# Chrixtar/latentsplat

Measured on AMD Instinct MI355X. Metric: rendered target views/sec at 256x256, ~300k Gaussians (forward); fwd+bwd ms/view in `fwdbwd`, higher is better.
Workload: dtype f32; 1 GPU; BASELINE configs[1]: 300000 latent Gaussians (4-ch features + opacity), 256x256, forward render; 16 views of one scene per step per GPU; gaussians=300000, parallelism=replicas x1 (one scene per rank, no data-path collective)

## Files before the change

latentsplat_amd/csrc/binning.hip:

```cpp
#include "lsr_blend.h"
#include "lsr_tile_scan.h"
#include <algorithm>
#include <mutex>
#ifdef LSR_ENABLE_TRACE
#include <cstdio>
#include <cstdlib>
#include <vector>
#endif

namespace lsr {

constexpr int kScanThreads = 1024;

constexpr int kScanRegs = 8;

__global__ void __launch_bounds__(kScanThreads)
k_tile_scan(const uint32_t *__restrict__ count, uint32_t *__restrict__ start, uint32_t *header,
            uint32_t *host_words, uint32_t host_seq, uint32_t *__restrict__ order, int N, uint32_t capacity) {
    __shared__ TileScanShared<kScanThreads> s_scan;
    tile_scan_block<kScanThreads, kScanRegs, false>(count, start, header, HostMirror{host_words, host_seq}, order, N, capacity, s_scan);
}

hipError_t launch_tile_scan(const lsr_dims &d, char *geom, uint32_t *host_words, uint32_t host_seq, uint32_t pair_capacity, hipStream_t s) {
    const GeomLayout L = geom_layout(d);
    const int N = d.num_views * (int)num_tiles(d);
    prof_begin(kStTileScan, s);
    hipLaunchKernelGGL(k_tile_scan, dim3(1), dim3(kScanThreads), 0, s,
                       (const uint32_t *)(geom + L.tile_count), (uint32_t *)(geom + L.tile_start),
                       (uint32_t *)(geom + L.header), host_words, host_seq, (uint32_t *)(geom + L.tile_order), N, pair_capacity);
    prof_end(kStTileScan, s);
    return hipGetLastError();
}

constexpr int kScatThreads = 256;
constexpr int kScatItems = 12;

template <bool LDS_RESERVE, bool NARROW>
__global__ void __launch_bounds__(kScatThreads, NARROW ? 8 : 6)
k_scatter(int G, int gx, int T, const char *__restrict__ binrec,
          const uint32_t *__restrict__ tile_start, uint32_t *__restrict__ tile_cursor,
          uint64_t *__restrict__ keys, uint32_t capacity, uint32_t chunks, int items, uint32_t key_shift, unsigned long long *trace,
          const uint32_t *__restrict__ tile_count, const uint32_t *__restrict__ header, uint32_t over_cap, int skip_none) {
    if (over_cap && header[kHdrMaxTile] <= over_cap) return;
#ifdef LSR_ENABLE_TRACE
#define LSR_STAMP(k) do { if (trace && threadIdx.x == 0) trace[8 * (size_t)blockIdx.x + (k)] = wall_clock64(); } while (0)
#else
#define LSR_STAMP(k) do { } while (0)
#endif
    LSR_STAMP(0);
    extern __shared__ uint32_t s_mem[];
    uint32_t *s_cnt = s_mem, *s_base = s_mem + T;
    const uint32_t unit = blockIdx.x;
    const int v = (int)(unit / chunks);
    const size_t vo = (size_t)v * G;
    const uint32_t *ts = tile_start + (size_t)v * T;
    uint32_t *cur = tile_cursor + (size_t)v * T;
    const uint32_t *tcv = tile_count + (size_t)v * T;
    const int base = (int)(unit % chunks) * (kScatThreads * items);
    uint32_t lo16[kScatItems], hi16[NARROW ? 1 : kScatItems], span[kScatItems];
    float dep[kScatItems];
#pragma unroll
    for (int it = 0; it < kScatItems; ++it) {
        const int i = base + min(it, items - 1) * kScatThreads + (int)threadIdx.x;
        const bool valid = it < items && i < G;
        if (NARROW) {
            const uint3 br = *(const uint3 *)(binrec + (vo + min(i, G - 1)) * sizeof(BinRec));
            lo16[it] = valid ? br.x : 0u; dep[it] = __uint_as_float(br.y); span[it] = br.z;
        } else {
            const uint4 br = *(const uint4 *)(binrec + (vo + min(i, G - 1)) * sizeof(BinRecWide));
            lo16[it] = br.x; hi16[NARROW ? 0 : it] = valid ? br.y : 0u; dep[it] = __uint_as_float(br.z); span[it] = br.w;
        }
    }
    auto unpack = [&](int it, int &x0, int &y0, int &x1, int &y1) {
        uint32_t a = lo16[it], b = NARROW ? 0u : hi16[NARROW ? 0 : it];
        asm volatile("" : "+v"(a), "+v"(b));
        if (NARROW) { x0 = a & 0xff; y0 = (a >> 8) & 0xff; x1 = (a >> 16) & 0xff; y1 = a >> 24; }
        else { x0 = a & 0xffff; y0 = a >> 16; x1 = b & 0xffff; y1 = b >> 16; }
    };
    if (LDS_RESERVE) {
        for (int t = threadIdx.x; t < T; t += kScatThreads) s_cnt[t] = 0;
        __syncthreads();
        LSR_STAMP(1);
#pragma unroll
        for (int it = 0; it < kScatItems; ++it) {
            int x0, y0, x1, y1;
            unpack(it, x0, y0, x1, y1);
            if (skip_none) reached_rect(span[it], x0, y0, x1, y1);
            for (int y = y0; y < y1; ++y)
                for (int x = x0; x < x1; ++x) {
                    if (over_cap && tcv[y * gx + x] <= over_cap) continue;
                    atomicAdd(&s_cnt[y * gx + x], 1u);
                }
        }
        __syncthreads();
        LSR_STAMP(2);
        for (int t = threadIdx.x; t < T; t += kScatThreads) {
            const uint32_t c = s_cnt[t];
            if (c) s_base[t] = ts[t] + atomicAdd(&cur[t], c);
            s_cnt[t] = 0;
        }
        __syncthreads();
        LSR_STAMP(3);
    }
    uint32_t tid2 = threadIdx.x;
    asm volatile("" : "+v"(tid2));
#pragma unroll
    for (int it = 0; it < kScatItems; ++it) {
        const uint32_t i = (uint32_t)(base + it * kScatThreads) + tid2;
        int x0, y0, x1, y1;
        unpack(it, x0, y0, x1, y1);
        if (x1 <= x0 || y1 <= y0) continue;
        const uint64_t key = ((uint64_t)__float_as_uint(dep[it]) << 32) | (i << key_shift);
        const uint32_t sp = span[it];
        int ex0 = x0, ey0 = y0, ex1 = x1, ey1 = y1;
        if (skip_none) reached_rect(sp, ex0, ey0, ex1, ey1);
        for (int y = ey0; y < ey1; ++y)
            for (int x = ex0; x < ex1; ++x) {
                const int t = y * gx + x;
                if (over_cap && tcv[t] <= over_cap) continue;
                const uint32_t code = key_shift ? span_code(sp, x - x0, y - y0) : 0u;
                uint32_t pos;
                if (LDS_RESERVE) pos = s_base[t] + atomicAdd(&s_cnt[t], 1u);
                else pos = ts[t] + atomicAdd(&cur[t], 1u);
                keys[min(pos, capacity - 1u)] = key | code;
            }
    }
    LSR_STAMP(4);
#ifdef LSR_ENABLE_TRACE
    __builtin_amdgcn_s_waitcnt(0);
    __syncthreads();
    LSR_STAMP(5);
    if (trace && threadIdx.x == 0) {
        unsigned hwid, xcc;
        asm volatile("s_getreg_b32 %0, hwreg(HW_REG_HW_ID)" : "=s"(hwid));
        asm volatile("s_getreg_b32 %0, hwreg(HW_REG_XCC_ID)" : "=s"(xcc));
        trace[8 * (size_t)blockIdx.x + 7] = ((unsigned long long)(xcc & 0xff) << 32) | hwid;
    }
#endif
#undef LSR_STAMP
}

constexpr int kSortThreads = 512;

struct HalfOut {
    uint32_t *half_list, *half_count;
    uint32_t *header;
    uint32_t capacity;
    uint32_t *long_list;
    uint32_t long_cap;
    uint32_t *long_count[2];
    IndexPacking ip;
    uint32_t seg_cap;
    const uint64_t *seg_keys;
    uint32_t n_limit;
};
constexpr int kSortTier2 = 8192;
__device__ __forceinline__ uint32_t long_tile(const HalfOut &ho, int cls, uint32_t i) {
    return ho.long_list[cls ? ho.long_cap - 1u - i : i];
}
__device__ __forceinline__ uint32_t key_index(const HalfOut &ho, uint32_t low_word) { return low_word >> ho.ip.key_shift; }
__device__ __forceinline__ uint32_t key_mask(const HalfOut &ho, uint32_t low_word) { return ho.ip.key_shift ? code_mask(low_word & 0xFFu) : 0xFFFFu; }
__device__ __forceinline__ uint32_t list_entry(const HalfOut &ho, uint32_t idx, uint32_t bits) { return idx | ((bits << kListBitsShift) & ~ho.ip.index_mask); }
constexpr int kEmitTab = 130;

template <int THREADS, class LowWord>
__device__ __forceinline__ void emit_half_lists(const HalfOut &ho, uint32_t n, uint32_t *hdst, uint32_t *hcnt, uint64_t *s_tab, LowWord low_word) {
    const int tid = threadIdx.x, lane = tid & (LSR_WAVE - 1), wid = tid / LSR_WAVE;
    constexpr int kWaves = THREADS / LSR_WAVE;
    uint32_t run0 = 0u, run1 = 0u;
    for (uint32_t base = 0; base < n; base += LSR_WAVE * LSR_WAVE) {
        for (int c = wid; c < LSR_WAVE; c += kWaves) {
            const uint32_t p = base + (uint32_t)(c * LSR_WAVE + lane);
            uint64_t packed = 0;
            if (p - lane < n) {
                const uint32_t w = low_word(min(p, n - 1));
                const uint32_t m16 = p < n ? key_mask(ho, w) : 0u;
                packed = (uint64_t)__builtin_popcountll(__ballot((m16 & 0x00FFu) != 0u)) |
                         ((uint64_t)__builtin_popcountll(__ballot((m16 & 0xFF00u) != 0u)) << 32);
            }
            if (lane == 0) s_tab[c] = packed;
        }
        __syncthreads();
        if (wid == 0) {
            const uint64_t v = s_tab[lane];
            uint64_t incl = v;
#pragma unroll
            for (int off = 1; off < LSR_WAVE; off <<= 1) { const uint64_t t = __shfl_up(incl, off); if (lane >= off) incl += t; }
            s_tab[LSR_WAVE + lane] = incl - v;
            if (lane == LSR_WAVE - 1) s_tab[2 * LSR_WAVE] = incl;
        }
        __syncthreads();
        const uint64_t tot = s_tab[2 * LSR_WAVE];
        for (int c = wid; c < LSR_WAVE; c += kWaves) {
            const uint32_t p = base + (uint32_t)(c * LSR_WAVE + lane);
            if (p - lane >= n) break;
            const uint32_t w = low_word(min(p, n - 1));
            const uint32_t idx = key_index(ho, w), m16 = p < n ? key_mask(ho, w) : 0u;
            const uint64_t off = s_tab[LSR_WAVE + c];
#pragma unroll
            for (int h = 0; h < 2; ++h) {
                const uint32_t bits = half_bits(m16, h);
                const uint64_t bal = __ballot(bits != 0u);
                if (bits) {
                    const uint32_t below = __builtin_amdgcn_mbcnt_hi((uint32_t)(bal >> 32), __builtin_amdgcn_mbcnt_lo((uint32_t)bal, 0u));
                    hdst[(size_t)h * n + (h ? run1 : run0) + (uint32_t)(off >> (32 * h)) + below] = list_entry(ho, idx, bits);
                }
            }
        }
        run0 += (uint32_t)tot; run1 += (uint32_t)(tot >> 32);
        __syncthreads();
    }
    if (tid < 2) hcnt[tid] = tid == 0 ? run0 : run1;
}

constexpr uint32_t kBucketOverflow = 48;

template <int CAP, int THREADS>
__device__ __forceinline__ void sort_tile(uint64_t *s_keys, size_t vt, int tier, const uint32_t *__restrict__ tile_start,
                                          const uint64_t *__restrict__ keys, uint32_t *__restrict__ point_list,
                                          const HalfOut &ho, unsigned long long *trace) {
#ifdef LSR_ENABLE_TRACE
#define LSR_STAMP(k) do { if (trace && threadIdx.x == 0) trace[8 * (size_t)blockIdx.x + (k)] = wall_clock64(); } while (0)
#else
#define LSR_STAMP(k) do { } while (0)
#endif
    LSR_STAMP(0);
    static_assert(CAP % THREADS == 0, "whole keys per thread");
    constexpr int NB = CAP < 2048 ? CAP : 2048;
    constexpr int kWaves = THREADS / LSR_WAVE;
    uint32_t *s_cnt = (uint32_t *)(s_keys + CAP);
    uint64_t *s_red = s_keys;
    uint32_t *s_wsum = (uint32_t *)(s_keys + 2 * kWaves);
    uint32_t *s_flag = s_wsum + kWaves;
    const int tid = threadIdx.x, lane = tid & (LSR_WAVE - 1), wid = tid / LSR_WAVE;
    const uint32_t start = tile_start[vt], n = tile_start[vt + 1] - start;
    uint32_t *hcnt = ho.half_count + 2 * vt, *hdst = ho.half_list + 2 * (size_t)start;
    if (n == 0) { if (tid < 2) hcnt[tid] = 0; return; }
    if ((uint64_t)start + n > ho.capacity) {
        if (tid < 2) hcnt[tid] = 0;
        if (tid == 0) ho.header[kHdrOverflow] = 1u;
        return;
    }
    if (n > ho.n_limit) {
        if (tid < 2) hcnt[tid] = 0;
        return;
    }
    if (n > (uint32_t)CAP) {
        if (tid == 0 && tier == 0) {
            const int cls = n > (uint32_t)kSortTier2 ? 1 : 0;
            const uint32_t i = atomicAdd(ho.long_count[cls], 1u);
            ho.long_list[cls ? ho.long_cap - 1u - i : i] = (uint32_t)vt;
        }
        return;
    }
    const uint64_t *src = (ho.seg_cap && n <= ho.seg_cap) ? ho.seg_keys + vt * (size_t)ho.seg_cap : keys + start;
    if (n == 1) {
        if (tid == 0) {
            const uint32_t w = (uint32_t)src[0], idx = key_index(ho, w);
            point_list[start] = idx;
            const uint32_t m = key_mask(ho, w);
            for (int h = 0; h < 2; ++h) {
                const uint32_t bits = half_bits(m, h);
                if (bits) hdst[h] = list_entry(ho, idx, bits);
                hcnt[h] = bits ? 1u : 0u;
            }
        }
        return;
    }

    constexpr int PERK = CAP / THREADS;
    uint64_t kreg[PERK];
#pragma unroll
    for (int q = 0; q < PERK; ++q) {
        const uint32_t i = tid + q * THREADS;
        const uint64_t k = src[min(i, n - 1)];
        kreg[q] = i < n ? k : ~0ull;
    }
    uint64_t kmin = ~0ull, kmax = 0ull;
#pragma unroll
    for (int q = 0; q < PERK; ++q) {
        const uint64_t k = kreg[q];
        kmin = k < kmin ? k : kmin;
        if (tid + q * THREADS < n) kmax = k > kmax ? k : kmax;
    }
#pragma unroll
    for (int off = 32; off > 0; off >>= 1) {
        const uint64_t a = __shfl_xor(kmin, off), b = __shfl_xor(kmax, off);
        kmin = a < kmin ? a : kmin; kmax = b > kmax ? b : kmax;
    }
    if (lane == 0) { s_red[2 * wid] = kmin; s_red[2 * wid + 1] = kmax; }
    for (int b = tid; b < NB; b += THREADS) s_cnt[b] = 0;
    if (tid == 0) *s_flag = 0;
    __syncthreads();
#pragma unroll
    for (int w = 0; w < kWaves; ++w) {
        kmin = s_red[2 * w] < kmin ? s_red[2 * w] : kmin;
        kmax = s_red[2 * w + 1] > kmax ? s_red[2 * w + 1] : kmax;
    }
    LSR_STAMP(1);
    const uint64_t range = kmax - kmin;
    const int bits = range ? 64 - __builtin_clzll(range) : 0;
    constexpr int LOGNB = NB == 4096 ? 12 : (NB == 2048 ? 11 : 10);
    const int shift = bits > LOGNB ? bits - LOGNB : 0;

    uint32_t rnk[PERK];
#pragma unroll
    for (int q = 0; q < PERK; ++q)
        if (tid + q * THREADS < n) rnk[q] = atomicAdd(&s_cnt[(uint32_t)((kreg[q] - kmin) >> shift)], 1u);
    __syncthreads();
    LSR_STAMP(2);
    constexpr int PER = (NB + THREADS - 1) / THREADS;
    uint32_t loc[PER], sum = 0, mx = 0;
#pragma unroll
    for (int q = 0; q < PER; ++q) {
        loc[q] = (NB % THREADS == 0 || tid * PER + q < NB) ? s_cnt[min(tid * PER + q, NB - 1)] : 0u;
        sum += loc[q]; mx = loc[q] > mx ? loc[q] : mx;
    }
    uint32_t incl = sum;
#pragma unroll
    for (int off = 1; off < LSR_WAVE; off <<= 1) { const uint32_t t = __shfl_up(incl, off); if (lane >= off) incl += t; }
    if (lane == LSR_WAVE - 1) s_wsum[wid] = incl;
    if (mx > kBucketOverflow) *s_flag = 1;
    __syncthreads();
    uint32_t run = incl - sum;
#pragma unroll
    for (int w = 0; w < kWaves; ++w) run += w < wid ? s_wsum[w] : 0u;
    const bool overflow = *s_flag != 0;
    if (!overflow) {
#pragma unroll
        for (int q = 0; q < PER; ++q) { if (NB % THREADS == 0 || tid * PER + q < NB) s_cnt[tid * PER + q] = run; run += loc[q]; }
        __syncthreads();
        LSR_STAMP(3);
#pragma unroll
        for (int q = 0; q < PERK; ++q)
            if (tid + q * THREADS < n) s_keys[s_cnt[(uint32_t)((kreg[q] - kmin) >> shift)] + rnk[q]] = kreg[q];
        __syncthreads();
        LSR_STAMP(4);
        uint32_t dst[PERK];
#pragma unroll
        for (int q = 0; q < PERK; ++q) {
            dst[q] = 0;
            if (tid + q * THREADS < n) {
                const uint64_t key = kreg[q];
                const uint32_t b = (uint32_t)((key - kmin) >> shift);
                const uint32_t lo = s_cnt[b], hi = b + 1 < (uint32_t)NB ? s_cnt[b + 1] : n;
                uint32_t below = 0;
                for (uint32_t j = lo; j < hi; j += 4) {
                    const uint32_t last = hi - 1;
                    const uint64_t m0 = s_keys[j], m1 = s_keys[min(j + 1, last)], m2 = s_keys[min(j + 2, last)], m3 = s_keys[min(j + 3, last)];
                    below += (m0 < key) + (j + 1 < hi && m1 < key) + (j + 2 < hi && m2 < key) + (j + 3 < hi && m3 < key);
                }
                dst[q] = lo + below;
            }
        }
        __syncthreads();
        uint32_t *s_out = (uint32_t *)s_keys;
#pragma unroll
        for (int q = 0; q < PERK; ++q)
            if (tid + q * THREADS < n) s_out[dst[q]] = (uint32_t)kreg[q];
        __syncthreads();
        LSR_STAMP(5);
        for (uint32_t i = tid; i < n; i += THREADS) point_list[start + i] = key_index(ho, s_out[i]);
        emit_half_lists<THREADS>(ho, n, hdst, hcnt, (uint64_t *)s_cnt, [&](uint32_t p) { return s_out[p]; });
        LSR_STAMP(6);
    } else {
        uint32_t npad = 2;
        while (npad < n) npad <<= 1;
        __syncthreads();
        if (npad <= (uint32_t)CAP) {
#pragma unroll
            for (int q = 0; q < PERK; ++q)
                if (tid + q * THREADS < npad) s_keys[tid + q * THREADS] = kreg[q];
        } else {
            static_assert(CAP * 8 + NB * 4 >= (CAP <= 2048 ? CAP : (CAP <= 4096 ? 4096 : CAP)) * 8, "bitonic padding fits the allocation");
#pragma unroll
            for (int q = 0; q < PERK; ++q) s_keys[tid + q * THREADS] = kreg[q];
            for (uint32_t i = CAP + tid; i < npad; i += THREADS) s_keys[i] = ~0ull;
        }
        __syncthreads();
        for (uint32_t k = 2; k <= npad; k <<= 1) {
            for (uint32_t j = k >> 1; j > 0; j >>= 1) {
                for (uint32_t t = tid; t < (npad >> 1); t += THREADS) {
                    const uint32_t lo = ((t & ~(j - 1)) << 1) | (t & (j - 1));
                    const uint32_t hi = lo | j;
                    const bool up = (lo & k) == 0;
                    const uint64_t a = s_keys[lo], b = s_keys[hi];
                    if ((a > b) == up) { s_keys[lo] = b; s_keys[hi] = a; }
                }
                __syncthreads();
            }
        }
        for (uint32_t i = tid; i < n; i += THREADS) point_list[start + i] = key_index(ho, (uint32_t)s_keys[i]);
        emit_half_lists<THREADS>(ho, n, hdst, hcnt, (uint64_t *)s_cnt, [&](uint32_t p) { return (uint32_t)s_keys[p]; });
    }
#ifdef LSR_ENABLE_TRACE
    if (trace && tid == 0) {
        unsigned hwid, xcc;
        asm volatile("s_getreg_b32 %0, hwreg(HW_REG_HW_ID)" : "=s"(hwid));
        asm volatile("s_getreg_b32 %0, hwreg(HW_REG_XCC_ID)" : "=s"(xcc));
        trace[8 * (size_t)blockIdx.x + 7] = ((unsigned long long)n << 40) | ((unsigned long long)(xcc & 0xff) << 32) | hwid;
    }
#endif
#undef LSR_STAMP
}

template <int CAP, int THREADS, bool PERSISTENT>
__global__ void __launch_bounds__(THREADS, CAP <= 4096 ? 6 : (CAP <= 8192 ? 4 : 2))
k_sort_tiles(int cls, const uint32_t *__restrict__ order, const uint32_t *__restrict__ tile_start, const uint64_t *__restrict__ keys,
             uint32_t *__restrict__ point_list, HalfOut ho, unsigned long long *trace) {
    extern __shared__ uint64_t s_keys[];
    if (!PERSISTENT) {
        const size_t vt = order ? (size_t)(order[2 * (size_t)blockIdx.x] & kItemTileMask) : (size_t)blockIdx.x;
        sort_tile<CAP, THREADS>(s_keys, vt, 0, tile_start, keys, point_list, ho, trace);
    } else {
        const uint32_t count = *ho.long_count[cls];
        for (uint32_t i = blockIdx.x; i < count; i += gridDim.x) {
            sort_tile<CAP, THREADS>(s_keys, long_tile(ho, cls, i), 1, tile_start, keys, point_list, ho, trace);
            __syncthreads();
        }
    }
}

__device__ __forceinline__ uint32_t lower_bound_u64(const uint64_t *a, uint32_t n, uint64_t x) {
    uint32_t lo = 0, hi = n;
    while (lo < hi) { const uint32_t mid = (lo + hi) >> 1; if (a[mid] < x) lo = mid + 1; else hi = mid; }
    return lo;
}
__device__ __forceinline__ void sort_tile_global(size_t vt, const uint32_t *__restrict__ tile_start, uint64_t *keys, uint64_t *tmp,
                                                 uint32_t *point_list, const HalfOut &ho, uint64_t *s_tab) {
    const uint32_t start = tile_start[vt], n = tile_start[vt + 1] - start;
    uint64_t *src = keys + start, *dst = tmp + start;
    for (uint32_t w = 1; w < n; w <<= 1) {
        for (uint32_t i = threadIdx.x; i < n; i += kSortThreads) {
            const uint32_t pair = i / (2 * w), a0 = pair * 2 * w;
            const uint32_t a1 = min(a0 + w, n), b1 = min(a0 + 2 * w, n);
            const uint64_t x = src[i];
            uint32_t pos;
            if (i < a1) pos = a0 + (i - a0) + lower_bound_u64(src + a1, b1 - a1, x);
            else pos = a0 + (i - a1) + lower_bound_u64(src + a0, a1 - a0, x);
            dst[pos] = x;
        }
        __threadfence_block();
        __syncthreads();
        uint64_t *t = src; src = dst; dst = t;
    }
    for (uint32_t i = threadIdx.x; i < n; i += kSortThreads)
        point_list[start + i] = key_index(ho, (uint32_t)src[i]);
    const uint64_t *sorted = src;
    emit_half_lists<kSortThreads>(ho, n, ho.half_list + 2 * (size_t)start, ho.half_count + 2 * vt, s_tab, [&](uint32_t p) { return (uint32_t)sorted[p]; });
}
__global__ void __launch_bounds__(kSortThreads)
k_sort_tiles_global(const uint32_t *__restrict__ tile_start, uint64_t *keys, uint64_t *tmp, uint32_t *point_list, HalfOut ho) {
    __shared__ uint64_t s_tab[kEmitTab];
    const uint32_t count = *ho.long_count[1];
    for (uint32_t it = blockIdx.x; it < count; it += gridDim.x) {
        const size_t vt = long_tile(ho, 1, it);
        if (tile_start[vt + 1] - tile_start[vt] <= (uint32_t)kSortLdsMax) continue;
        sort_tile_global(vt, tile_start, keys, tmp, point_list, ho, s_tab);
        __syncthreads();
    }
}
__global__ void __launch_bounds__(kSortThreads, 2)
k_sort_tiles_long(const uint32_t *__restrict__ tile_start, uint64_t *keys, uint64_t *tmp, uint32_t *point_list, HalfOut ho) {
    extern __shared__ uint64_t s_keys[];
    const uint32_t c0 = *ho.long_count[0], c1 = *ho.long_count[1];
    for (uint32_t it = blockIdx.x; it < c0 + c1; it += gridDim.x) {
        const size_t vt = it < c0 ? long_tile(ho, 0, it) : long_tile(ho, 1, it - c0);
        if (tile_start[vt + 1] - tile_start[vt] <= (uint32_t)kSortLdsMax) sort_tile<kSortLdsMax, kSortThreads>(s_keys, vt, 1, tile_start, keys, point_list, ho, nullptr);
        else sort_tile_global(vt, tile_start, keys, tmp, point_list, ho, s_keys);
        __syncthreads();
    }
}

template <int CAP>
constexpr size_t sort_lds_bytes() { return (size_t)CAP * 8 + (size_t)(CAP < 2048 ? CAP : 2048) * 4; }
template <int CAP, int THREADS, bool PERS>
static void sort_launch(dim3 grid, hipStream_t s, int cls, const uint32_t *order, const uint32_t *ts, const uint64_t *keys,
                        uint32_t *plist, const HalfOut &ho, unsigned long long *trace) {
    constexpr size_t lds = sort_lds_bytes<CAP>();
    if (lds > 48 * 1024) {
        static uint64_t done = 0;
        static std::mutex mu;
        int dev = 0;
        (void)hipGetDevice(&dev);
        std::lock_guard<std::mutex> lock(mu);
        if (dev < 0 || dev >= 64 || !((done >> dev) & 1ull)) {
            (void)hipFuncSetAttribute((const void *)k_sort_tiles<CAP, THREADS, PERS>, hipFuncAttributeMaxDynamicSharedMemorySize, (int)lds);
            if (dev >= 0 && dev < 64) done |= 1ull << dev;
        }
    }
    hipLaunchKernelGGL((k_sort_tiles<CAP, THREADS, PERS>), grid, dim3(THREADS), lds, s, cls, order, ts, keys, plist, ho, trace);
}

hipError_t launch_binning(const lsr_dims &d, char *geom, char *bin, int64_t num_pairs,
                          int32_t max_tile_pairs, const int32_t *radii, hipStream_t s, bool device_counts, bool seg, bool speculative) {
    (void)radii;
    const GeomLayout L = geom_layout(d);
    if (num_pairs <= 0 || d.num_gaussians == 0)
        return launch_clear(geom + L.half_count, align_up((size_t)d.num_views * (size_t)num_tiles(d) * 8, 16), s);
    const BinLayout B = bin_layout(d, num_pairs, device_counts ? kSortLdsMax + 1 : max_tile_pairs);
    const int T = (int)num_tiles(d), gx = tiles_x(d);
    if (seg && L.seg_cap == 0) return hipErrorInvalidValue;
    uint64_t *keys = (uint64_t *)(bin + B.keys);
    uint32_t *plist = (uint32_t *)(bin + B.point_list);
    const uint32_t *ts = (const uint32_t *)(geom + L.tile_start);
    HalfOut ho;
    ho.half_list = (uint32_t *)(bin + B.half_list); ho.half_count = (uint32_t *)(geom + L.half_count);
    ho.header = (uint32_t *)(geom + L.header);
    ho.capacity = (uint32_t)(num_pairs < 0xFFFFFFFFll ? num_pairs : 0xFFFFFFFFll);
    ho.long_list = (uint32_t *)(geom + L.tile_cursor);
    ho.long_cap = (uint32_t)d.num_views * (uint32_t)T;
    ho.long_count[0] = ho.header + kHdrLongTiles; ho.long_count[1] = ho.long_count[0] + 1;
    ho.ip = index_packing(d);
    ho.seg_cap = seg ? L.seg_cap : 0u;
    ho.seg_keys = (const uint64_t *)(geom + L.seg_keys);
    ho.n_limit = speculative ? (uint32_t)max_tile_pairs : 0xFFFFFFFFu;
    const uint32_t over_cap = seg ? L.seg_cap : 0u;
    if (!seg || device_counts || (uint32_t)max_tile_pairs > L.seg_cap) {
        const bool lds = T <= 8192;
        const int64_t resident = (int64_t)device_cus() * (lds ? std::max<int64_t>(1, std::min<int64_t>(8, (160 * 1024) / ((int64_t)T * 8 + 64))) : 8);
        const int64_t work = (int64_t)d.num_views * d.num_gaussians;
        const int64_t rounds = (work + resident * kScatThreads * kScatItems - 1) / (resident * kScatThreads * kScatItems);
        int items = (int)((work + resident * kScatThreads * rounds - 1) / (resident * kScatThreads * rounds));
        const int min_items = (int)((d.num_gaussians + (int64_t)kScatThreads * 160 - 1) / ((int64_t)kScatThreads * 160));
        items = std::max(1, std::min(kScatItems, std::max(items, min_items)));
        const uint32_t chunks = (uint32_t)((d.num_gaussians + kScatThreads * items - 1) / (kScatThreads * items));
        dim3 grid(chunks * (uint32_t)d.num_views);
        unsigned long long *strace = nullptr;
#ifdef LSR_ENABLE_TRACE
        const char *strace_path = getenv("LSR_TRACE_SCATTER");
        if (strace_path) {
            (void)hipMalloc((void **)&strace, (size_t)grid.x * 64);
            (void)hipMemsetAsync(strace, 0, (size_t)grid.x * 64, s);
        }
#endif
        prof_begin(kStScatter, s);
        const uint32_t capacity = (uint32_t)(num_pairs < 0xFFFFFFFFll ? num_pairs : 0xFFFFFFFFll);
#define LSR_SCAT2(LDSR, NRW, SHM)                                                                         \
    hipLaunchKernelGGL((k_scatter<LDSR, NRW>), grid, dim3(kScatThreads), SHM, s, d.num_gaussians, gx, T, \
                       (const char *)(geom + L.bin), ts, (uint32_t *)(geom + L.tile_cursor), keys, capacity, chunks, items, index_packing(d).key_shift, strace, \
                       (const uint32_t *)(geom + L.tile_count), (const uint32_t *)(geom + L.header), over_cap, reached_only(d) ? 1 : 0)
#define LSR_SCAT(LDSR, SHM) do { if (narrow_bins(d)) LSR_SCAT2(LDSR, true, SHM); else LSR_SCAT2(LDSR, false, SHM); } while (0)
        if (lds) LSR_SCAT(true, (size_t)T * 8);
        else LSR_SCAT(false, 0);
#undef LSR_SCAT
#undef LSR_SCAT2
        prof_end(kStScatter, s);
#ifdef LSR_ENABLE_TRACE
        if (strace_path) {
            std::vector<unsigned long long> host((size_t)grid.x * 8);
            (void)hipStreamSynchronize(s);
            (void)hipMemcpy(host.data(), strace, host.size() * 8, hipMemcpyDeviceToHost);
            if (FILE *f = fopen(strace_path, "wb")) { fwrite(host.data(), 8, host.size(), f); fclose(f); }
            (void)hipFree(strace);
        }
#endif
        hipError_t e = hipGetLastError();
        if (e != hipSuccess) return e;
    }
    {
        dim3 grid((uint32_t)T * (uint32_t)d.num_views);
        unsigned long long *trace = nullptr;
#ifdef LSR_ENABLE_TRACE
        const char *trace_path = getenv("LSR_TRACE_SORT");
        if (trace_path) {
            (void)hipMalloc((void **)&trace, (size_t)grid.x * 64);
            (void)hipMemsetAsync(trace, 0, (size_t)grid.x * 64, s);
        }
#endif
        prof_begin(kStSort, s);
        const uint32_t *order = env_int("LSR_SORT_LPT", 1) ? (const uint32_t *)(geom + L.tile_order) : nullptr;
        const int32_t longest = device_counts ? std::max<int32_t>(max_tile_pairs, 4096) : max_tile_pairs;
        int32_t tier1;
        if (longest <= 1024) { tier1 = 1024; sort_launch<1024, 512, false>(grid, s, 0, order, ts, keys, plist, ho, trace); }
        else if (longest <= 2048) { tier1 = 2048; sort_launch<2048, 512, false>(grid, s, 0, order, ts, keys, plist, ho, trace); }
        else { tier1 = 4096; sort_launch<4096, 512, false>(grid, s, 0, order, ts, keys, plist, ho, trace); }
        hipError_t e = hipGetLastError();
        if (e != hipSuccess) return e;
        const uint32_t cus = (uint32_t)device_cus();
        const dim3 pgrid(cus);
        if (device_counts) {
            constexpr size_t lds = sort_lds_bytes<kSortLdsMax>();
            static uint64_t attr_done = 0;
            static std::mutex attr_mu;
            int dev = 0;
            (void)hipGetDevice(&dev);
            {
                std::lock_guard<std::mutex> lock(attr_mu);
                if (dev < 0 || dev >= 64 || !((attr_done >> dev) & 1ull)) {
                    (void)hipFuncSetAttribute((const void *)k_sort_tiles_long, hipFuncAttributeMaxDynamicSharedMemorySize, (int)lds);
                    if (dev >= 0 && dev < 64) attr_done |= 1ull << dev;
                }
            }
            hipLaunchKernelGGL(k_sort_tiles_long, pgrid, dim3(kSortThreads), lds, s, ts, keys, (uint64_t *)(bin + B.tmp), plist, ho);
            e = hipGetLastError();
            if (e != hipSuccess) return e;
        } else {
        if (max_tile_pairs > tier1) {
            sort_launch<kSortTier2, 512, true>(dim3(2 * cus), s, 0, nullptr, ts, keys, plist, ho, trace);
            e = hipGetLastError();
            if (e != hipSuccess) return e;
        }
        if (max_tile_pairs > kSortTier2) {
            sort_launch<kSortLdsMax, 512, true>(pgrid, s, 1, nullptr, ts, keys, plist, ho, trace);
            e = hipGetLastError();
            if (e != hipSuccess) return e;
        }
        if (max_tile_pairs > kSortLdsMax) {
            hipLaunchKernelGGL(k_sort_tiles_global, pgrid, dim3(kSortThreads), 0, s, ts, keys, (uint64_t *)(bin + B.tmp), plist, ho);
            e = hipGetLastError();
            if (e != hipSuccess) return e;
        }
        }
        prof_end(kStSort, s);
#ifdef LSR_ENABLE_TRACE
        if (trace_path) {
            std::vector<unsigned long long> host((size_t)grid.x * 8);
            (void)hipStreamSynchronize(s);
            (void)hipMemcpy(host.data(), trace, host.size() * 8, hipMemcpyDeviceToHost);
            if (FILE *f = fopen(trace_path, "wb")) { fwrite(host.data(), 8, host.size(), f); fclose(f); }
            (void)hipFree(trace);
        }
#endif
    }
    return hipSuccess;
}

}
```

Before: 40840 views/s.

## Speed up per-tile sort: DPP reductions, early-exit key loops, LDS mask table

```diff
diff --git a/latentsplat_amd/csrc/binning.hip b/latentsplat_amd/csrc/binning.hip
--- a/latentsplat_amd/csrc/binning.hip
+++ b/latentsplat_amd/csrc/binning.hip
@@ -161,12 +161,23 @@
 __device__ __forceinline__ uint32_t key_index(const HalfOut &ho, uint32_t low_word) { return low_word >> ho.ip.key_shift; }
 __device__ __forceinline__ uint32_t key_mask(const HalfOut &ho, uint32_t low_word) { return ho.ip.key_shift ? code_mask(low_word & 0xFFu) : 0xFFFFu; }
 __device__ __forceinline__ uint32_t list_entry(const HalfOut &ho, uint32_t idx, uint32_t bits) { return idx | ((bits << kListBitsShift) & ~ho.ip.index_mask); }
-constexpr int kEmitTab = 130;
+constexpr int kEmitScan = 130;
+constexpr int kEmitTab = kEmitScan + 64;
+
+template <int THREADS>
+__device__ __forceinline__ void build_mask_table(const HalfOut &ho, uint64_t *s_tab) {
+    uint16_t *s_mask = (uint16_t *)(s_tab + kEmitScan);
+    if (ho.ip.key_shift)
+        for (int c = threadIdx.x; c < 256; c += THREADS) s_mask[c] = (uint16_t)code_mask((uint32_t)c);
+}
 
 template <int THREADS, class LowWord>
 __device__ __forceinline__ void emit_half_lists(const HalfOut &ho, uint32_t n, uint32_t *hdst, uint32_t *hcnt, uint64_t *s_tab, LowWord low_word) {
     const int tid = threadIdx.x, lane = tid & (LSR_WAVE - 1), wid = tid / LSR_WAVE;
     constexpr int kWaves = THREADS / LSR_WAVE;
+    const uint16_t *s_mask = (const uint16_t *)(s_tab + kEmitScan);
+    const bool coded = ho.ip.key_shift != 0;
+    auto mask_of = [&](uint32_t w) -> uint32_t { return coded ? (uint32_t)s_mask[w & 0xFFu] : 0xFFFFu; };
     uint32_t run0 = 0u, run1 = 0u;
     for (uint32_t base = 0; base < n; base += LSR_WAVE * LSR_WAVE) {
         for (int c = wid; c < LSR_WAVE; c += kWaves) {
@@ -174,7 +185,7 @@
             uint64_t packed = 0;
             if (p - lane < n) {
                 const uint32_t w = low_word(min(p, n - 1));
-                const uint32_t m16 = p < n ? key_mask(ho, w) : 0u;
+                const uint32_t m16 = p < n ? mask_of(w) : 0u;
                 packed = (uint64_t)__builtin_popcountll(__ballot((m16 & 0x00FFu) != 0u)) |
                          ((uint64_t)__builtin_popcountll(__ballot((m16 & 0xFF00u) != 0u)) << 32);
             }
@@ -195,7 +206,7 @@
             const uint32_t p = base + (uint32_t)(c * LSR_WAVE + lane);
             if (p - lane >= n) break;
             const uint32_t w = low_word(min(p, n - 1));
-            const uint32_t idx = key_index(ho, w), m16 = p < n ? key_mask(ho, w) : 0u;
+            const uint32_t idx = key_index(ho, w), m16 = p < n ? mask_of(w) : 0u;
             const uint64_t off = s_tab[LSR_WAVE + c];
 #pragma unroll
             for (int h = 0; h < 2; ++h) {
@@ -213,6 +224,26 @@
     if (tid < 2) hcnt[tid] = tid == 0 ? run0 : run1;
 }
 
+template <int CTRL> __device__ __forceinline__ uint32_t dpp_u32(uint32_t x) { return (uint32_t)__builtin_amdgcn_update_dpp(0, (int)x, CTRL, 0xf, 0xf, false); }
+#define LSR_ROW_REDUCE(name, op)                                                                        \
+    __device__ __forceinline__ uint32_t name(uint32_t x) {                                              \
+        x = op(x, dpp_u32<0xB1>(x));                                           \
+        x = op(x, dpp_u32<0x4E>(x));                                           \
+        x = op(x, dpp_u32<0x141>(x));                                              \
+        return op(x, dpp_u32<0x140>(x));                                                \
+    }
+__device__ __forceinline__ uint32_t add_u32(uint32_t a, uint32_t b) { return a + b; }
+__device__ __forceinline__ uint32_t min_u32(uint32_t a, uint32_t b) { return a < b ? a : b; }
+__device__ __forceinline__ uint32_t max_u32(uint32_t a, uint32_t b) { return a > b ? a : b; }
+LSR_ROW_REDUCE(row_min_u32, min_u32)
+LSR_ROW_REDUCE(row_max_u32, max_u32)
+LSR_ROW_REDUCE(row_sum_u32, add_u32)
+#undef LSR_ROW_REDUCE
+__device__ __forceinline__ uint32_t rdlane(uint32_t x, int l) { return (uint32_t)__builtin_amdgcn_readlane((int)x, l); }
+__device__ __forceinline__ uint64_t uniform_u64(uint64_t x) {
+    return ((uint64_t)(uint32_t)__builtin_amdgcn_readfirstlane((int)(x >> 32)) << 32) | (uint32_t)__builtin_amdgcn_readfirstlane((int)(uint32_t)x);
+}
+
 constexpr uint32_t kBucketOverflow = 48;
 
 template <int CAP, int THREADS>
@@ -229,8 +260,10 @@
     constexpr int NB = CAP < 2048 ? CAP : 2048;
     constexpr int kWaves = THREADS / LSR_WAVE;
     uint32_t *s_cnt = (uint32_t *)(s_keys + CAP);
-    uint64_t *s_red = s_keys;
-    uint32_t *s_wsum = (uint32_t *)(s_keys + 2 * kWaves);
+    static_assert(kWaves <= 16 && (kWaves & (kWaves - 1)) == 0, "cross-wave partials are reduced inside one DPP row");
+    uint2 *s_red32 = (uint2 *)s_keys;
+    uint64_t *s_red = s_keys + kWaves;
+    uint32_t *s_wsum = (uint32_t *)(s_keys + 3 * kWaves);
     uint32_t *s_flag = s_wsum + kWaves;
     const int tid = threadIdx.x, lane = tid & (LSR_WAVE - 1), wid = tid / LSR_WAVE;
     const uint32_t start = tile_start[vt], n = tile_start[vt + 1] - start;
@@ -269,33 +302,56 @@
     }
 
     constexpr int PERK = CAP / THREADS;
+    const int nq = __builtin_amdgcn_readfirstlane((int)((n + THREADS - 1) / THREADS));
+    constexpr bool kEarly = PERK <= 8;
+#define LSR_LIVE(q) if (kEarly && (q) >= nq) break
     uint64_t kreg[PERK];
 #pragma unroll
     for (int q = 0; q < PERK; ++q) {
-        const uint32_t i = tid + q * THREADS;
-        const uint64_t k = src[min(i, n - 1)];
-        kreg[q] = i < n ? k : ~0ull;
-    }
-    uint64_t kmin = ~0ull, kmax = 0ull;
-#pragma unroll
-    for (int q = 0; q < PERK; ++q) {
-        const uint64_t k = kreg[q];
-        kmin = k < kmin ? k : kmin;
-        if (tid + q * THREADS < n) kmax = k > kmax ? k : kmax;
-    }
-#pragma unroll
-    for (int off = 32; off > 0; off >>= 1) {
-        const uint64_t a = __shfl_xor(kmin, off), b = __shfl_xor(kmax, off);
-        kmin = a < kmin ? a : kmin; kmax = b > kmax ? b : kmax;
-    }
-    if (lane == 0) { s_red[2 * wid] = kmin; s_red[2 * wid + 1] = kmax; }
+        LSR_LIVE(q);
+        kreg[q] = src[min((uint32_t)(tid + q * THREADS), n - 1)];
+    }
     for (int b = tid; b < NB; b += THREADS) s_cnt[b] = 0;
     if (tid == 0) *s_flag = 0;
+    uint64_t kmin, kmax;
+    uint32_t dmin = ~0u, dmax = 0u;
+#pragma unroll
+    for (int q = 0; q < PERK; ++q) {
+        LSR_LIVE(q);
+        const uint32_t dw = (uint32_t)(kreg[q] >> 32);
+        dmin = min(dmin, dw); dmax = max(dmax, dw);
+    }
+    dmin = row_min_u32(dmin); dmax = row_max_u32(dmax);
+    const uint32_t wmin = min(min(rdlane(dmin, 0), rdlane(dmin, 16)), min(rdlane(dmin, 32), rdlane(dmin, 48)));
+    const uint32_t wmax = max(max(rdlane(dmax, 0), rdlane(dmax, 16)), max(rdlane(dmax, 32), rdlane(dmax, 48)));
+    if (lane == 0) s_red32[wid] = make_uint2(wmin, wmax);
     __syncthreads();
-#pragma unroll
-    for (int w = 0; w < kWaves; ++w) {
-        kmin = s_red[2 * w] < kmin ? s_red[2 * w] : kmin;
-        kmax = s_red[2 * w + 1] > kmax ? s_red[2 * w + 1] : kmax;
+    const uint2 part = s_red32[lane & (kWaves - 1)];
+    dmin = (uint32_t)__builtin_amdgcn_readfirstlane((int)row_min_u32(part.x));
+    dmax = (uint32_t)__builtin_amdgcn_readfirstlane((int)row_max_u32(part.y));
+    kmin = (uint64_t)dmin << 32; kmax = ((uint64_t)dmax << 32) | 0xFFFFFFFFull;
+    const bool exact = dmax - dmin < (uint32_t)NB;
+    if (exact) {
+        uint64_t lo = ~0ull, hi = 0ull;
+#pragma unroll
+        for (int q = 0; q < PERK; ++q) {
+            LSR_LIVE(q);
+            const uint64_t k = kreg[q];
+            lo = k < lo ? k : lo; hi = k > hi ? k : hi;
+        }
+#pragma unroll
+        for (int off = 32; off > 0; off >>= 1) {
+            const uint64_t a = __shfl_xor(lo, off), b = __shfl_xor(hi, off);
+            lo = a < lo ? a : lo; hi = b > hi ? b : hi;
+        }
+        if (lane == 0) { s_red[2 * wid] = lo; s_red[2 * wid + 1] = hi; }
+        __syncthreads();
+#pragma unroll
+        for (int w = 0; w < kWaves; ++w) {
+            lo = s_red[2 * w] < lo ? s_red[2 * w] : lo;
+            hi = s_red[2 * w + 1] > hi ? s_red[2 * w + 1] : hi;
+        }
+        kmin = uniform_u64(lo); kmax = uniform_u64(hi);
     }
     LSR_STAMP(1);
     const uint64_t range = kmax - kmin;
@@ -305,8 +361,10 @@
 
     uint32_t rnk[PERK];
 #pragma unroll
-    for (int q = 0; q < PERK; ++q)
+    for (int q = 0; q < PERK; ++q) {
+        LSR_LIVE(q);
         if (tid + q * THREADS < n) rnk[q] = atomicAdd(&s_cnt[(uint32_t)((kreg[q] - kmin) >> shift)], 1u);
+    }
     __syncthreads();
     LSR_STAMP(2);
     constexpr int PER = (NB + THREADS - 1) / THREADS;
@@ -323,8 +381,10 @@
     if (mx > kBucketOverflow) *s_flag = 1;
     __syncthreads();
     uint32_t run = incl - sum;
-#pragma unroll
-    for (int w = 0; w < kWaves; ++w) run += w < wid ? s_wsum[w] : 0u;
+    {
+        const uint32_t mine = s_wsum[lane & (kWaves - 1)];
+        run += (uint32_t)__builtin_amdgcn_readfirstlane((int)row_sum_u32(lane < wid ? mine : 0u));
+    }
     const bool overflow = *s_flag != 0;
     if (!overflow) {
 #pragma unroll
@@ -332,15 +392,17 @@
         __syncthreads();
         LSR_STAMP(3);
 #pragma unroll
-        for (int q = 0; q < PERK; ++q)
+        for (int q = 0; q < PERK; ++q) {
+            LSR_LIVE(q);
             if (tid + q * THREADS < n) s_keys[s_cnt[(uint32_t)((kreg[q] - kmin) >> shift)] + rnk[q]] = kreg[q];
+        }
         __syncthreads();
         LSR_STAMP(4);
         uint32_t dst[PERK];
 #pragma unroll
         for (int q = 0; q < PERK; ++q) {
             dst[q] = 0;
-            if (tid + q * THREADS < n) {
+            if ((!kEarly || q < nq) && tid + q * THREADS < n) {
                 const uint64_t key = kreg[q];
                 const uint32_t b = (uint32_t)((key - kmin) >> shift);
                 const uint32_t lo = s_cnt[b], hi = b + 1 < (uint32_t)NB ? s_cnt[b + 1] : n;
@@ -356,8 +418,11 @@
         __syncthreads();
         uint32_t *s_out = (uint32_t *)s_keys;
 #pragma unroll
-        for (int q = 0; q < PERK; ++q)
+        for (int q = 0; q < PERK; ++q) {
+            LSR_LIVE(q);
             if (tid + q * THREADS < n) s_out[dst[q]] = (uint32_t)kreg[q];
+        }
+        build_mask_table<THREADS>(ho, (uint64_t *)s_cnt);
         __syncthreads();
         LSR_STAMP(5);
         for (uint32_t i = tid; i < n; i += THREADS) point_list[start + i] = key_index(ho, s_out[i]);
@@ -367,16 +432,13 @@
         uint32_t npad = 2;
         while (npad < n) npad <<= 1;
         __syncthreads();
-        if (npad <= (uint32_t)CAP) {
-#pragma unroll
-            for (int q = 0; q < PERK; ++q)
-                if (tid + q * THREADS < npad) s_keys[tid + q * THREADS] = kreg[q];
-        } else {
-            static_assert(CAP * 8 + NB * 4 >= (CAP <= 2048 ? CAP : (CAP <= 4096 ? 4096 : CAP)) * 8, "bitonic padding fits the allocation");
-#pragma unroll
-            for (int q = 0; q < PERK; ++q) s_keys[tid + q * THREADS] = kreg[q];
-            for (uint32_t i = CAP + tid; i < npad; i += THREADS) s_keys[i] = ~0ull;
-        }
+        static_assert(CAP * 8 + NB * 4 >= (CAP <= 2048 ? CAP : (CAP <= 4096 ? 4096 : CAP)) * 8, "bitonic padding fits the allocation");
+#pragma unroll
+        for (int q = 0; q < PERK; ++q) {
+            LSR_LIVE(q);
+            if (tid + q * THREADS < n) s_keys[tid + q * THREADS] = kreg[q];
+        }
+        for (uint32_t i = n + tid; i < npad; i += THREADS) s_keys[i] = ~0ull;
         __syncthreads();
         for (uint32_t k = 2; k <= npad; k <<= 1) {
             for (uint32_t j = k >> 1; j > 0; j >>= 1) {
@@ -390,6 +452,8 @@
                 __syncthreads();
             }
         }
+        build_mask_table<THREADS>(ho, (uint64_t *)s_cnt);
+        __syncthreads();
         for (uint32_t i = tid; i < n; i += THREADS) point_list[start + i] = key_index(ho, (uint32_t)s_keys[i]);
         emit_half_lists<THREADS>(ho, n, hdst, hcnt, (uint64_t *)s_cnt, [&](uint32_t p) { return (uint32_t)s_keys[p]; });
     }
@@ -401,6 +465,7 @@
         trace[8 * (size_t)blockIdx.x + 7] = ((unsigned long long)n << 40) | ((unsigned long long)(xcc & 0xff) << 32) | hwid;
     }
 #endif
+#undef LSR_LIVE
 #undef LSR_STAMP
 }
 
@@ -447,6 +512,8 @@
     for (uint32_t i = threadIdx.x; i < n; i += kSortThreads)
         point_list[start + i] = key_index(ho, (uint32_t)src[i]);
     const uint64_t *sorted = src;
+    build_mask_table<kSortThreads>(ho, s_tab);
+    __syncthreads();
     emit_half_lists<kSortThreads>(ho, n, ho.half_list + 2 * (size_t)start, ho.half_count + 2 * vt, s_tab, [&](uint32_t p) { return (uint32_t)sorted[p]; });
 }
 __global__ void __launch_bounds__(kSortThreads)
```

Result: faster. 41850 views/s (median of 6 runs) (+2.5%).
